# brdav/refign

Measured on AMD Instinct MI355X. Metric: image-pairs/s (align+seg fwd+bwd, 1080x1920), higher is better.
Workload: dtype bf16

## Files before the change

### include/refign_hip.h

```cpp
#ifndef REFIGN_HIP_H
#define REFIGN_HIP_H

#ifdef __cplusplus
extern "C" {
#endif

#define RFN_OK 0
#define RFN_EINVAL (-1)
#define RFN_ELAUNCH (-2)
#define RFN_ENOTSUP (-3)
#define RFN_ENONDET (-4)

#define RFN_ABI_VERSION 5

typedef void* rfn_stream_t;

int rfn_abi_version(void);
const char* rfn_last_error(void);

int rfn_set_deterministic(int on);
int rfn_get_deterministic(void);

int rfn_corr_fwd_f32(const float* in1, const float* in2, float* out, int B, int C, int iH, int iW,
                     int kH, int kW, int patchH, int patchW, int padH, int padW, int dilH, int dilW,
// ... 220 lines not shown
int rfn_dacs_blur(const float* x, float* tmp, float* y, int B, int C, int H, int W, int ksize_y, int ksize_x, const int* blur_on,
                  const double* sigma_y, const double* sigma_x, rfn_stream_t stream);

int rfn_crop_label_hist_u8(const void* label, int H, int W, const int* boxes, int K, int* hist, rfn_stream_t stream);
int rfn_crop_flip_norm_u8(const void* image, const void* label, int C, int H, int W, int top, int left, int h, int w, int flip,
                          const float* mean3, const float* std3, float* out_image, long* out_label, rfn_stream_t stream);

int rfn_resize_crop_flip_norm_u8(const void* image_hwc, int H, int W, int Hd, int Wd, const int* bounds_x, const int* coef_x, int kmax_x,
                                 const int* bounds_y, const int* coef_y, int kmax_y, int top, int left, int h, int w, int flip,
                                 const float* mean3, const float* std3, float* out_image, rfn_stream_t stream);
int rfn_resize_u8(const void* image_hwc, int H, int W, int Hd, int Wd, const int* bounds_x, const int* coef_x, int kmax_x,
                  const int* bounds_y, const int* coef_y, int kmax_y, void* out_chw, rfn_stream_t stream);
int rfn_resize_nearest_u8(const void* label, int H, int W, int Hd, int Wd, const int* ytab, const int* xtab, void* out,
                          rfn_stream_t stream);

int rfn_resize_filter_u8(const void* image_hwc, int H, int W, int Hd, int Wd, int filter, const int* bounds_x, const int* coef_x,
                         int kmax_x, const int* bounds_y, const int* coef_y, int kmax_y, void* out_chw, rfn_stream_t stream);
int rfn_resize_filter_crop_flip_norm_pad_u8(const void* image_hwc, int H, int W, int Hd, int Wd, int filter, const int* bounds_x,
                                            const int* coef_x, int kmax_x, const int* bounds_y, const int* coef_y, int kmax_y, int top,
                                            int left, int h, int w, int flip, const float* mean3, const float* std3, float* out_image,
                                            int Hf, int Wf, rfn_stream_t stream);

int rfn_sparse_epe_f32(const float* flow, const float* conf, const float* pts_src, const float* pts_trg, const int* offsets, int B,
                       int h, int w, double* rows, rfn_stream_t stream);

int rfn_gemm_nt_f8(const void* X8, const void* W8, const float* wscale, float x_scale, const void* bias, const void* res,
                   const float* rowscale, int rows_per_sample, int act, void* Y, int out_f8, float out_q, long M, long N,
                   long K, long ldx, long ldw, long ldy, rfn_stream_t stream);
int rfn_quant_rows_f8(const void* table, int nchunks, rfn_stream_t stream);
int rfn_quant_f8(const void* x_bf16, void* y8, long n, float q, rfn_stream_t stream);
int rfn_layernorm_fwd_f8(const void* x_bf16, const float* gamma, const float* beta, void* y8, long rows, int C, float eps,
                         float out_q, rfn_stream_t stream);
int rfn_dwconv3x3_gelu_nhwc_fwd_f8(const void* x8, const float* weight, const float* bias, void* y8, int B, int H, int W, int C,
                                   float x_scale, float out_q, rfn_stream_t stream);
int rfn_attn_pack_f8(const void* kv8, long batch_stride, long row_stride, int B, int heads, int Nkv, int nst, void* pack,
                     rfn_stream_t stream);
int rfn_attn_fwd_f8(const void* q8, long q_batch_stride, long q_row_stride, const void* pack, void* o8, long o_batch_stride,
                    long o_row_stride, int B, int heads, int Nq, int Nkv, int nst, float scale, float q_scale, float k_scale,
                    float v_scale, float out_q, rfn_stream_t stream);

unsigned long rfn_bn_stats_det_workspace_bytes(long T, int C);
int rfn_bn_stats_fwd_det(const void* x, double* sums, void* workspace, long T, int C, int dtype, rfn_stream_t stream);
int rfn_bn_stats_bwd_det(const void* x, const void* grad_y, const double* fwd_sums, const float* gamma, const float* beta,
                         float* bwd_sums, void* workspace, long T, int C, float eps, int relu, int dtype, rfn_stream_t stream);
unsigned long rfn_dwconv3x3_stats_det_workspace_bytes(int B, int H, int W, int C, int dilation);
int rfn_dwconv3x3_nhwc_fwd_stats_det(const void* x, const float* weight, const float* bias, void* y, double* sums, void* workspace,
                                     int B, int H, int W, int C, int dilation, int dtype, rfn_stream_t stream);
int rfn_dwconv3x3_nhwc_stats_det(const void* x, const float* weight, const float* bias, double* sums, void* workspace, int B, int H,
                                 int W, int C, int dilation, int dtype, rfn_stream_t stream);
int rfn_attn_bwd_dkv_det(const void* K, const void* V, long kv_batch_stride, long kv_row_stride, const void* q_rpack,
                         const void* q_tpack, const void* do_rpack, const void* do_tpack, const float* lse2,
                         const float* delta, float* accT, void* dKV, int B, int heads, int Nq, int Nkv, int nqblk, int nqpad,
                         int nkpad, int blocks_per_chunk, float scale, int dtype, rfn_stream_t stream);
unsigned long rfn_dacs_mix_jitter_det_workspace_bytes(int H, int W);
int rfn_dacs_mix_jitter_det(const float* src, const float* trg, const long* gt_src, const long* pseudo_label,
                            const float* pseudo_weight, float* mixed_img, long* mixed_lbl, float* mixed_weight, double* mean_ws,
                            int B, int H, int W, const long* class_bits, const int* jitter_on, const int* order,
                            const float* factor, const float* hue, const float* mean3, const float* std3,
                            rfn_stream_t stream);
unsigned long rfn_upsample_ce_det_workspace_bytes(int B, int C, int H, int W);
int rfn_upsample_ce_det(const void* logits, const long* target, const float* weight, float* grad_lo, double* loss_sum,
                        void* workspace, int B, int C, int h, int w, int H, int W, int ignore_index, int dtype, int round16,
                        rfn_stream_t stream);
int rfn_upsample_bilinear2d_bwd(const void* grad_out, void* grad_in, long planes, int h, int w, int H, int W, float scale_y,
                                float scale_x, int dtype, rfn_stream_t stream);

int rfn_steplog_gather(const void* const* ptrs, const int* dtypes, int n, double* row, rfn_stream_t stream);
int rfn_grad_sqnorm_groups(const float* flat, long n, const long* chunks, int nchunks, int ngroups, double* partials,
                           double* out, rfn_stream_t stream);

int rfn_flowsynth_flow_f32(const float* theta, int kind, const float* bumps, int n_bumps, const float* field, int h, int w,
                           float* flow, int* count, rfn_stream_t stream);
int rfn_flowsynth_warp_f32(const float* image, const float* flow, const int* count, int h, int w, int top, int left, int ch, int cw,
                           double min_fraction_valid, float* out_image, float* out_flow, void* out_mask, rfn_stream_t stream);
int rfn_gaussian_blur_f32(const float* src, const float* taps, int ntaps, int planes, int h, int w, double* tmp, float* dst,
                          rfn_stream_t stream);

int rfn_flowloss_block_pixels(void);
int rfn_flowloss_fwd_f32(const float* gt_flow, int B, int H, int W, const long* levels, const double* weights, int nlevels,
                         int loss_type, float delta, double* partials, int nblocks, float* loss_out, double* counts,
                         rfn_stream_t stream);
int rfn_flowloss_bwd_f32(const float* gt_flow, int B, int H, int W, const long* levels, const double* weights, int nlevels,
                         int loss_type, float delta, const double* counts, const float* grad_out, rfn_stream_t stream);
int rfn_multi_adam_f32(const void* table, int nchunks, const float* group_args, int ngroups, rfn_stream_t stream);
int rfn_multi_adam_amp_f32(const void* table, int nchunks, const double* group_args, int ngroups, const float* found_inf,
                           const float* step, rfn_stream_t stream);

int rfn_photometric_record_words(void);
int rfn_photometric_gray_sums_u8(const void* image, const void* records, int B, int h, int w, unsigned long* sums,
                                 rfn_stream_t stream);
int rfn_photometric_apply_u8(const void* image, const void* records, const unsigned long* sums, int B, int h, int w, float* out,
                             rfn_stream_t stream);

int rfn_rotate_nearest_u8(const void* src, int C, int H, int W, int a0, int a1, int a2, int a3, int a4, int a5, int fill,
                          void* out, void* outside, rfn_stream_t stream);
int rfn_photometric_gray_sums_geom_u8(const void* image, const void* records, const void* geom, int B, int H, int W, int h, int w,
                                      unsigned long* sums, rfn_stream_t stream);
int rfn_photometric_apply_geom_u8(const void* image, const void* records, const void* geom, const unsigned long* sums, int B, int H,
                                  int W, int h, int w, float* out, rfn_stream_t stream);

unsigned long rfn_warp_bwd_det_workspace_bytes(int B, int C, int H, int W, int want_grad_x, int want_grad_flow);
int rfn_warp_bwd_det_f32(const float* x, const float* flow, const float* grad_out, float* grad_x, float* grad_flow,
                         void* workspace, int B, int C, int H, int W, rfn_stream_t stream);
int rfn_corr_bwd_gather_f32(const float* in1, const float* in2, const float* grad_out, float* grad_in1,
                            float* grad_in2, int B, int C, int iH, int iW, int kH, int kW, int patchH, int patchW,
                            int padH, int padW, int dilH, int dilW, int dpH, int dpW, int dH, int dW,
// ... 7 lines not shown
```

### refign_amd/csrc/attn.hip

```cpp
#include <cstdlib>

#include "common.h"
#include "mfma.h"

namespace rfn {

constexpr int kPackBlock = 4096;
constexpr float kLog2e = 1.4426950408889634f;

__global__ __launch_bounds__(256) void attn_pack_kernel(const uint16_t* __restrict__ src0, const uint16_t* __restrict__ src1,
                                                        long sb, long sr, int heads, int nrows, int nblk,
                                                        unsigned char* __restrict__ rpack0, unsigned char* __restrict__ tpack0,
                                                        unsigned char* __restrict__ rpack1, unsigned char* __restrict__ tpack1) {
  __shared__ unsigned tile[32][33];
  const uint16_t* src = blockIdx.z ? src1 : src0;
  unsigned char* rpack = blockIdx.z ? rpack1 : rpack0;
  unsigned char* tpack = blockIdx.z ? tpack1 : tpack0;
  const int blk = blockIdx.x, bh = blockIdx.y;
  const int b = bh / heads, hd = bh % heads;
  const int t = threadIdx.x, row = t >> 3, dc = t & 7;
  const int grow = blk * 32 + row;
  u32x4 v = {0u, 0u, 0u, 0u};
  if (grow < nrows) v = *(const u32x4*)(src + (long)b * sb + (long)grow * sr + hd * 64 + dc * 8);
  unsigned char* rb = rpack + ((long)bh * nblk + blk) * kPackBlock;
// ... 144 lines not shown
      for (int kb = 0; kb < 2; ++kb)
#pragma unroll
        for (int r = 0; r < 16; ++r)
          if (key0 + kb * 32 + (r & 3) + 8 * (r >> 2) + 4 * g >= Nkv) p[kb][r] = -1e30f;
    }
    float mt = p[0][0];
#pragma unroll
    for (int kb = 0; kb < 2; ++kb)
#pragma unroll
      for (int r = 0; r < 16; ++r) mt = fmaxf(mt, p[kb][r]);
    mt = half_max(mt) * c;
    const float mnew = fmaxf(mrun, mt);
    if (__any(mnew > mrun)) {
      const float alpha = __builtin_amdgcn_exp2f(mrun - mnew);
      lrun *= alpha;
#pragma unroll
      for (int r = 0; r < 16; ++r) {
        oacc[0][r] *= alpha;
        oacc[1][r] *= alpha;
      }
      mrun = mnew;
    }
    float ps = 0.f;
#pragma unroll
    for (int kb = 0; kb < 2; ++kb)
#pragma unroll
      for (int r = 0; r < 16; ++r) {
        p[kb][r] = __builtin_amdgcn_exp2f(__builtin_fmaf(p[kb][r], c, -mrun));
        ps += p[kb][r];
      }
    lrun += ps;
    {
      vec8 pb[2][2];
      to_operands<DT>(p[0], pb[0]);
      to_operands<DT>(p[1], pb[1]);
#pragma unroll
      for (int idx = 0; idx < 8; ++idx) {
        const int kb = idx >> 2, m = (idx >> 1) & 1, db = idx & 1;
        oacc[db] = E::mma(vfr[idx & 3], pb[kb][m], oacc[db]);
        if (idx + 4 < 8) vfr[idx & 3] = vfrag(idx + 4);
        __builtin_amdgcn_sched_barrier(0);
      }
    }
    wait_dma_all();
    wg_barrier();
  }
  const float l = half_sum(lrun);
  const bool ok = q < Nq;
  store_rows64<DT>(oacc, 1.f / l, O + (long)b * osb + (long)(ok ? q : 0) * osr + hd * 64, ok, g);
  if (g == 0 && q < nqpad) lse2[(long)bh * nqpad + q] = ok ? mrun + log2f(l) : 0.f;
}


template <int DT>
__global__ __launch_bounds__(256) void attn_bwd_dq_kernel(const uint16_t* __restrict__ Q, long qsb, long qsr,
                                                          const uint16_t* __restrict__ dO, const uint16_t* __restrict__ O,
                                                          long osb, long osr, const unsigned char* __restrict__ Kr,
                                                          const unsigned char* __restrict__ Vr,
                                                          const unsigned char* __restrict__ Kt,
                                                          const float* __restrict__ lse2, float* __restrict__ delta,
                                                          uint16_t* __restrict__ dQ, long dsb, long dsr, int heads, int Nq,
                                                          int Nkv, int nblk, int nqpad, float scale, int pheads) {
  using E = Elem<DT>;
  using vec8 = typename E::vec8;
  constexpr int STAGE = 6 * kPackBlock;
  __shared__ __attribute__((aligned(16))) unsigned char smem[2 * STAGE];
  const int lane = threadIdx.x & 63, wave = threadIdx.x >> 6, g = lane >> 5, col = lane & 31;
  const int bh = blockIdx.y, b = bh / heads, hd = bh % heads;
  const int q = blockIdx.x * 128 + wave * 32 + col;
  const bool ok = q < Nq;
  const float c = scale * kLog2e;

  vec8 qf[4], gf[4];
  load_row_frags<DT>(Q + (long)b * qsb + hd * 64, qsr, q, Nq, g, qf);
  load_row_frags<DT>(dO + (long)b * osb + hd * 64, osr, q, Nq, g, gf);
  float dl = 0.f;
  {
    vec8 of[4];
    load_row_frags<DT>(O + (long)b * osb + hd * 64, osr, q, Nq, g, of);
#pragma unroll
    for (int kk = 0; kk < 4; ++kk)
#pragma unroll
      for (int e = 0; e < 8; ++e) dl += (float)gf[kk][e] * (float)of[kk][e];
    dl = half_sum(dl);
  }
  const float ls = (q < nqpad) ? lse2[(long)bh * nqpad + q] : 0.f;
  if (g == 0 && q < nqpad) delta[(long)bh * nqpad + q] = ok ? dl : 0.f;
#pragma unroll
  for (int kk = 0; kk < 4; ++kk) {
    pin_loaded(qf[kk]);
    pin_loaded(gf[kk]);
  }
  pin_loaded(ls);

  const long pbase = (long)(b * pheads + hd) * nblk * kPackBlock;
  const int nst = nblk / 2;
  auto issue = [&](int st, int buf) {
    unsigned char* dst = smem + buf * STAGE;
#pragma unroll
    for (int u = 0; u < 2; ++u) {
      const int piece = wave * 2 + u;
      const long off = pbase + (long)st * 2 * kPackBlock + piece * 1024 + lane * 16;
      lds_dma16(Kr + off, dst + piece * 1024);
      lds_dma16(Vr + off, dst + 2 * kPackBlock + piece * 1024);
      lds_dma16(Kt + off, dst + 4 * kPackBlock + piece * 1024);
    }
  };

  f32x16 dq[2];
#pragma unroll
  for (int r = 0; r < 16; ++r) dq[0][r] = dq[1][r] = 0.f;

  issue(0, 0);
  wait_dma_all();
  wg_barrier();
// ... 13 lines not shown
        const int kb = idx >> 3, kk = (idx >> 1) & 3;
        return *(const vec8*)(base + ((idx & 1) * 2 + kb) * kPackBlock + ((2 * kk + g) * 32 + col) * 16);
      };
#pragma unroll
      for (int idx = 0; idx < 4; ++idx) fr[idx] = frag(idx);
      __builtin_amdgcn_sched_barrier(0);
#pragma unroll
      for (int idx = 0; idx < 16; ++idx) {
        const int kb = idx >> 3, kk = (idx >> 1) & 3;
        if (idx & 1) dpacc[kb] = E::mma(fr[idx & 3], gf[kk], dpacc[kb]);
        else sacc[kb] = E::mma(fr[idx & 3], qf[kk], sacc[kb]);
        if (idx + 4 < 16) fr[idx & 3] = frag(idx + 4);
        __builtin_amdgcn_sched_barrier(0);
      }
    }
    vec8 ktf[4];
    auto ktfrag = [&](int idx) {
      const unsigned char* kq = base + (4 + (idx >> 2)) * kPackBlock + ((idx & 1) * 32 + col) * 8;
      const int m = (idx >> 1) & 1;
      return join8<DT>(*(const u32x2*)(kq + (4 * m + g) * 512), *(const u32x2*)(kq + (4 * m + 2 + g) * 512));
    };
#pragma unroll
    for (int idx = 0; idx < 4; ++idx) ktf[idx] = ktfrag(idx);
    __builtin_amdgcn_sched_barrier(0);
    float ds[2][16];
#pragma unroll
    for (int kb = 0; kb < 2; ++kb)
#pragma unroll
      for (int r = 0; r < 16; ++r)
        ds[kb][r] = __builtin_amdgcn_exp2f(__builtin_fmaf(sacc[kb][r], c, -ls)) * (dpacc[kb][r] - dl);
    if (key0 + 64 > Nkv) {
      asm volatile("; padded keys" ::: "memory");
#pragma unroll
      for (int kb = 0; kb < 2; ++kb)
#pragma unroll
        for (int r = 0; r < 16; ++r)
          if (key0 + kb * 32 + (r & 3) + 8 * (r >> 2) + 4 * g >= Nkv) ds[kb][r] = 0.f;
    }
    {
      vec8 sb[2][2];
      to_operands<DT>(ds[0], sb[0]);
      to_operands<DT>(ds[1], sb[1]);
#pragma unroll
      for (int idx = 0; idx < 8; ++idx) {
        dq[idx & 1] = E::mma(ktf[idx & 3], sb[idx >> 2][(idx >> 1) & 1], dq[idx & 1]);
        if (idx + 4 < 8) ktf[idx & 3] = ktfrag(idx + 4);
        __builtin_amdgcn_sched_barrier(0);
      }
    }
    wait_dma_all();
    wg_barrier();
  }
  store_rows64<DT>(dq, scale, dQ + (long)b * dsb + (long)(ok ? q : 0) * dsr + hd * 64, ok, g);
}

template <int DT, int NS>
__global__ __launch_bounds__(512) void attn_bwd_dkv_kernel(const uint16_t* __restrict__ K, const uint16_t* __restrict__ V,
                                                           long ksb, long ksr, const unsigned char* __restrict__ Qr,
                                                           const unsigned char* __restrict__ Qt,
                                                           const unsigned char* __restrict__ Gr,
                                                           const unsigned char* __restrict__ Gt,
                                                           const float* __restrict__ lse2, const float* __restrict__ delta,
                                                           float* __restrict__ accT, int heads, int Nq, int Nkv, int nqblk,
                                                           int nqpad, int nkpad, int blocks_per_chunk, float scale,
                                                           long chunk_stride = 0) {
  using E = Elem<DT>;
  using vec8 = typename E::vec8;
  constexpr int STATS = 4 * kPackBlock;
  constexpr int STAGE = STATS + 256;
  __shared__ __attribute__((aligned(16))) unsigned char smem[NS * STAGE];
  const int lane = threadIdx.x & 63, wave = threadIdx.x >> 6, g = lane >> 5, col = lane & 31;
  const int bh = blockIdx.z, b = bh / heads, hd = bh % heads;
  const int key = blockIdx.x * 256 + wave * 32 + col;
  const bool wave_live = blockIdx.x * 256 + wave * 32 < Nkv;
  const bool kok = key < Nkv;
  const float c = scale * kLog2e;

  vec8 kf[4], vf[4];
  load_row_frags<DT>(K + (long)b * ksb + hd * 64, ksr, key, Nkv, g, kf);
  load_row_frags<DT>(V + (long)b * ksb + hd * 64, ksr, key, Nkv, g, vf);
#pragma unroll
  for (int kk = 0; kk < 4; ++kk) {
    pin_loaded(kf[kk]);
    pin_loaded(vf[kk]);
  }

  const int qb0 = blockIdx.y * blocks_per_chunk;
  const int nst = min(qb0 + blocks_per_chunk, nqblk) - qb0;
  const long pbase = (long)bh * nqblk * kPackBlock;
  const float* stat_src = (g == 0 ? lse2 : delta) + (long)bh * nqpad + col;
  auto issue = [&](int qb, int buf) {
    unsigned char* dst = smem + buf * STAGE;
    const long off = pbase + (long)qb * kPackBlock + (wave & 3) * 1024 + lane * 16;
    if (wave < 4) {
      lds_dma16(Qr + off, dst + (wave & 3) * 1024);
      lds_dma16(Gr + off, dst + kPackBlock + (wave & 3) * 1024);
    } else {
      lds_dma16(Qt + off, dst + 2 * kPackBlock + (wave & 3) * 1024);
      lds_dma16(Gt + off, dst + 3 * kPackBlock + (wave & 3) * 1024);
    }
    if (wave == 0) lds_dma4(stat_src + qb * 32, dst + STATS);
  };

  f32x16 dk[2], dv[2];
#pragma unroll
  for (int r = 0; r < 16; ++r) dk[0][r] = dk[1][r] = dv[0][r] = dv[1][r] = 0.f;

#pragma unroll
  for (int s = 0; s < NS - 1; ++s)
    if (s < nst) issue(qb0 + s, s);
  for (int i = 0; i < nst; ++i) {
    if (NS == 2 || i + NS - 2 >= nst) wait_dma_all();
    else if (wave == 0) wait_dma_upto<(NS - 2) * 3>();
    else wait_dma_upto<(NS - 2) * 2>();
    wg_barrier();
    if (i + NS - 1 < nst) issue(qb0 + i + NS - 1, (i + NS - 1) % NS);
    if (wave_live) {
      const unsigned char* base = smem + (i % NS) * STAGE;
// ... 18 lines not shown
        for (int idx = 0; idx < 8; ++idx) {
          if (idx & 1) dp = E::mma(fr[idx & 3], vf[idx >> 1], dp);
          else s = E::mma(fr[idx & 3], kf[idx >> 1], s);
          if (idx + 4 < 8) fr[idx & 3] = frag(idx + 4);
          __builtin_amdgcn_sched_barrier(0);
        }
      }
      vec8 tf[4];
      auto tfrag = [&](int idx) {
        const int m = idx >> 2, db = (idx >> 1) & 1;
        const unsigned char* pq = base + (2 + ((idx & 1) ^ 1)) * kPackBlock + (db * 32 + col) * 8;
        return join8<DT>(*(const u32x2*)(pq + (4 * m + g) * 512), *(const u32x2*)(pq + (4 * m + 2 + g) * 512));
      };
#pragma unroll
      for (int idx = 0; idx < 4; ++idx) tf[idx] = tfrag(idx);
      __builtin_amdgcn_sched_barrier(0);
      float p[16], ds[16];
#pragma unroll
      for (int r = 0; r < 16; ++r) {
        float pr = __builtin_amdgcn_exp2f(__builtin_fmaf(s[r], c, -l4[r >> 2][r & 3]));
        if (!kok) pr = 0.f;
        p[r] = pr;
        ds[r] = pr * (dp[r] - d4[r >> 2][r & 3]);
      }
      vec8 pb[2], sb[2];
      to_operands<DT>(p, pb);
      to_operands<DT>(ds, sb);
#pragma unroll
      for (int idx = 0; idx < 8; ++idx) {
        const int m = idx >> 2, db = (idx >> 1) & 1;
        if (idx & 1) dk[db] = E::mma(tf[idx & 3], sb[m], dk[db]);
        else dv[db] = E::mma(tf[idx & 3], pb[m], dv[db]);
        if (idx + 4 < 8) tf[idx & 3] = tfrag(idx + 4);
        __builtin_amdgcn_sched_barrier(0);
      }
    }
  }
  if (kok) {
    float* ak = accT + (long)blockIdx.y * chunk_stride + (long)bh * 2 * 64 * nkpad + key;
    float* av = ak + (long)64 * nkpad;
#pragma unroll
    for (int db = 0; db < 2; ++db)
#pragma unroll
      for (int r = 0; r < 16; ++r) {
        const int d = db * 32 + (r & 3) + 8 * (r >> 2) + 4 * g;
        if (chunk_stride != 0) {
          ak[(long)d * nkpad] = dk[db][r] * scale;
          av[(long)d * nkpad] = dv[db][r];
        } else {
          atomicAdd(ak + (long)d * nkpad, dk[db][r] * scale);
          atomicAdd(av + (long)d * nkpad, dv[db][r]);
        }
      }
  }
}

template <int DT>
__global__ __launch_bounds__(256) void attn_dkv_finish_kernel(const float* __restrict__ accT, uint16_t* __restrict__ dkv,
                                                              int heads, int Nkv, int nkpad, long total, int chunks = 1,
                                                              long chunk_stride = 0) {
  using S = typename Elem<DT>::scalar;
  const long i = (long)blockIdx.x * 256 + threadIdx.x;
  if (i >= total) return;
  const int d = (int)(i & 63);
  long r = i >> 6;
  const int hd = (int)(r % heads);
  r /= heads;
  const int which = (int)(r & 1);
  r >>= 1;
  const int key = (int)(r % Nkv);
  const int b = (int)(r / Nkv);
  const float* p = accT + (((long)(b * heads + hd) * 2 + which) * 64 + d) * nkpad + key;
  float v = p[0];
  for (int c = 1; c < chunks; ++c) v += p[(long)c * chunk_stride];
  const S o = (S)v;
  dkv[i] = __builtin_bit_cast(uint16_t, o);
}

}

extern "C" {

using namespace rfn;

#define ATTN_DT_OK(dt) RFN_REQUIRE((dt) == 1 || (dt) == 2, "attention: dtype %d (1 = bf16, 2 = f16)", (dt))

int rfn_attn_pack(const void* src, long batch_stride, long row_stride, int B, int heads, int nrows, int nblk, void* rpack,
                  void* tpack, const void* src2, void* rpack2, void* tpack2, rfn_stream_t stream) {
  RFN_REQUIRE(src && (rpack || tpack), "attn_pack: null pointer");
  RFN_REQUIRE(src2 == nullptr || rpack2 || tpack2, "attn_pack: second tensor without outputs");
  RFN_REQUIRE(B > 0 && heads > 0 && nrows > 0 && nblk * 32 >= nrows, "attn_pack: B=%d heads=%d rows=%d nblk=%d", B, heads,
              nrows, nblk);
  RFN_REQUIRE(row_stride % 8 == 0 && batch_stride % 8 == 0, "attn_pack: strides must be multiples of 8 elements");
  dim3 grid(nblk, B * heads, src2 ? 2 : 1);
  hipLaunchKernelGGL(attn_pack_kernel, grid, dim3(256), 0, (hipStream_t)stream, (const uint16_t*)src,
                     (const uint16_t*)src2, batch_stride, row_stride, heads, nrows, nblk, (unsigned char*)rpack,
                     (unsigned char*)tpack, (unsigned char*)rpack2, (unsigned char*)tpack2);
  return check_launch("attn_pack");
}

int rfn_attn_fwd(const void* Q, long q_batch_stride, long q_row_stride, const void* k_rpack, const void* v_tpack, void* O,
                 long o_batch_stride, long o_row_stride, float* lse2, int B, int heads, int Nq, int Nkv, int nkblk,
                 int nqpad, float scale, int kv_pack_heads, int dtype, rfn_stream_t stream) {
  ATTN_DT_OK(dtype);
  RFN_REQUIRE(Q && k_rpack && v_tpack && O && lse2, "attn_fwd: null pointer");
  RFN_REQUIRE(B > 0 && heads > 0 && Nq > 0 && Nkv > 0 && nkblk % 2 == 0 && nkblk * 32 >= Nkv && nqpad >= Nq,
              "attn_fwd: B=%d heads=%d Nq=%d Nkv=%d nkblk=%d nqpad=%d", B, heads, Nq, Nkv, nkblk, nqpad);
  RFN_REQUIRE(q_row_stride % 8 == 0 && o_row_stride % 8 == 0 && q_batch_stride % 8 == 0 && o_batch_stride % 8 == 0,
              "attn_fwd: strides must be multiples of 8 elements");
  RFN_REQUIRE(kv_pack_heads >= heads, "attn_fwd: kv_pack_heads");
  dim3 grid(cdiv(Nq, 128), B * heads);
  if (dtype == 1)
    hipLaunchKernelGGL(attn_fwd_kernel<1>, grid, dim3(256), 0, (hipStream_t)stream, (const uint16_t*)Q, q_batch_stride,
                       q_row_stride, (const unsigned char*)k_rpack, (const unsigned char*)v_tpack, (uint16_t*)O,
                       o_batch_stride, o_row_stride, lse2, heads, Nq, Nkv, nkblk, nqpad, scale, kv_pack_heads);
  else
    hipLaunchKernelGGL(attn_fwd_kernel<2>, grid, dim3(256), 0, (hipStream_t)stream, (const uint16_t*)Q, q_batch_stride,
                       q_row_stride, (const unsigned char*)k_rpack, (const unsigned char*)v_tpack, (uint16_t*)O,
                       o_batch_stride, o_row_stride, lse2, heads, Nq, Nkv, nkblk, nqpad, scale, kv_pack_heads);
  return check_launch("attn_fwd");
}

int rfn_attn_bwd_dq(const void* Q, long q_batch_stride, long q_row_stride, const void* dO, const void* O,
                    long o_batch_stride, long o_row_stride, const void* k_rpack, const void* v_rpack, const void* k_tpack,
                    const float* lse2, float* delta, void* dQ, long dq_batch_stride, long dq_row_stride, int B, int heads,
                    int Nq, int Nkv, int nkblk, int nqpad, float scale, int kv_pack_heads, int dtype,
                    rfn_stream_t stream) {
  ATTN_DT_OK(dtype);
  RFN_REQUIRE(Q && dO && O && k_rpack && v_rpack && k_tpack && lse2 && delta && dQ, "attn_bwd_dq: null pointer");
  RFN_REQUIRE(B > 0 && heads > 0 && Nq > 0 && Nkv > 0 && nkblk % 2 == 0 && nkblk * 32 >= Nkv && nqpad >= Nq,
              "attn_bwd_dq: B=%d heads=%d Nq=%d Nkv=%d nkblk=%d nqpad=%d", B, heads, Nq, Nkv, nkblk, nqpad);
  dim3 grid(cdiv(Nq, 128), B * heads);
#define RFN_DQ_LAUNCH(D)                                                                                                \
  hipLaunchKernelGGL(attn_bwd_dq_kernel<D>, grid, dim3(256), 0, (hipStream_t)stream, (const uint16_t*)Q, q_batch_stride, \
                     q_row_stride, (const uint16_t*)dO, (const uint16_t*)O, o_batch_stride, o_row_stride,               \
                     (const unsigned char*)k_rpack, (const unsigned char*)v_rpack, (const unsigned char*)k_tpack, lse2,  \
                     delta, (uint16_t*)dQ, dq_batch_stride, dq_row_stride, heads, Nq, Nkv, nkblk, nqpad, scale,          \
                     kv_pack_heads)
  if (dtype == 1) RFN_DQ_LAUNCH(1); else RFN_DQ_LAUNCH(2);
#undef RFN_DQ_LAUNCH
  return check_launch("attn_bwd_dq");
}

static int attn_bwd_dkv_impl(bool det, const void* K, const void* V, long kv_batch_stride, long kv_row_stride, const void* q_rpack,
                             const void* q_tpack, const void* do_rpack, const void* do_tpack, const float* lse2,
                             const float* delta, float* accT, void* dKV, int B, int heads, int Nq, int Nkv, int nqblk, int nqpad,
                             int nkpad, int blocks_per_chunk, float scale, int dtype, rfn_stream_t stream) {
  ATTN_DT_OK(dtype);
  RFN_REQUIRE(K && V && q_rpack && q_tpack && do_rpack && do_tpack && lse2 && delta && accT && dKV,
              "attn_bwd_dkv: null pointer");
  RFN_REQUIRE(B > 0 && heads > 0 && Nq > 0 && Nkv > 0 && nqblk * 32 >= Nq && nqpad >= nqblk * 32 && nkpad >= Nkv &&
                  nkpad % 32 == 0 && blocks_per_chunk > 0,
              "attn_bwd_dkv: B=%d heads=%d Nq=%d Nkv=%d nqblk=%d nqpad=%d nkpad=%d chunk=%d", B, heads, Nq, Nkv, nqblk,
              nqpad, nkpad, blocks_per_chunk);
  hipStream_t s = (hipStream_t)stream;
  const long image = (long)B * heads * 2 * 64 * nkpad, chunk_stride = det ? image : 0;
  if (!det)
    if (int rc = zero_async(accT, (size_t)image * sizeof(float), s)) return rc;
  dim3 grid(cdiv(Nkv, 256), cdiv(nqblk, blocks_per_chunk), B * heads);
  const int chunks = det ? (int)grid.y : 1;
  static const int ring = 2;
#define RFN_DKV_LAUNCH_(D, R)                                                                                           \
  hipLaunchKernelGGL((attn_bwd_dkv_kernel<D, R>), grid, dim3(512), 0, s, (const uint16_t*)K, (const uint16_t*)V,            \
                     kv_batch_stride, kv_row_stride, (const unsigned char*)q_rpack, (const unsigned char*)q_tpack,      \
                     (const unsigned char*)do_rpack, (const unsigned char*)do_tpack, lse2, delta, accT, heads, Nq, Nkv,  \
                     nqblk, nqpad, nkpad, blocks_per_chunk, scale, chunk_stride)
#define RFN_DKV_LAUNCH(D)                                                                                               \
  switch (ring) {                                                                                                       \
    case 4: RFN_DKV_LAUNCH_(D, 4); break;                                                                               \
    default: RFN_DKV_LAUNCH_(D, 2); break;                                                                              \
  }
  if (dtype == 1) { RFN_DKV_LAUNCH(1) } else { RFN_DKV_LAUNCH(2) }
#undef RFN_DKV_LAUNCH
#undef RFN_DKV_LAUNCH_
  int rc = check_launch("attn_bwd_dkv");
  if (rc != RFN_OK) return rc;
  const long total = (long)B * Nkv * 2 * heads * 64;
  if (dtype == 1)
    hipLaunchKernelGGL(attn_dkv_finish_kernel<1>, dim3(cdiv(total, 256)), dim3(256), 0, s, accT, (uint16_t*)dKV, heads,
                       Nkv, nkpad, total, chunks, chunk_stride);
  else
    hipLaunchKernelGGL(attn_dkv_finish_kernel<2>, dim3(cdiv(total, 256)), dim3(256), 0, s, accT, (uint16_t*)dKV, heads,
                       Nkv, nkpad, total, chunks, chunk_stride);
  return check_launch("attn_dkv_finish");
}

int rfn_attn_bwd_dkv(const void* K, const void* V, long kv_batch_stride, long kv_row_stride, const void* q_rpack,
                     const void* q_tpack, const void* do_rpack, const void* do_tpack, const float* lse2,
                     const float* delta, float* accT, void* dKV, int B, int heads, int Nq, int Nkv, int nqblk, int nqpad,
                     int nkpad, int blocks_per_chunk, float scale, int dtype, rfn_stream_t stream) {
  RFN_REFUSE_NONDET(true, "rfn_attn_bwd_dkv", "attn_bwd_dkv_kernel, fp32 atomics (use rfn_attn_bwd_dkv_det)");
  return attn_bwd_dkv_impl(false, K, V, kv_batch_stride, kv_row_stride, q_rpack, q_tpack, do_rpack, do_tpack, lse2, delta, accT,
                           dKV, B, heads, Nq, Nkv, nqblk, nqpad, nkpad, blocks_per_chunk, scale, dtype, stream);
}

int rfn_attn_bwd_dkv_det(const void* K, const void* V, long kv_batch_stride, long kv_row_stride, const void* q_rpack,
                         const void* q_tpack, const void* do_rpack, const void* do_tpack, const float* lse2,
                         const float* delta, float* accT, void* dKV, int B, int heads, int Nq, int Nkv, int nqblk, int nqpad,
                         int nkpad, int blocks_per_chunk, float scale, int dtype, rfn_stream_t stream) {
  return attn_bwd_dkv_impl(true, K, V, kv_batch_stride, kv_row_stride, q_rpack, q_tpack, do_rpack, do_tpack, lse2, delta, accT,
                           dKV, B, heads, Nq, Nkv, nqblk, nqpad, nkpad, blocks_per_chunk, scale, dtype, stream);
}

}
```

### refign_amd/mfma.py

```python
import ctypes
import os

import torch

from . import _lib, determinism
from ._tensor import ptr
from ._tensor import DTYPE_CODE16 as _DT16

ENABLED = True

LIBRARY_CALLS = {}
_NOTE = True


def note_library(kind, *tensors):
    if not _NOTE or not tensors or not tensors[0].is_cuda:
        return
    key = (kind, str(tensors[0].dtype).replace("torch.", ""), tuple(tuple(t.shape) for t in tensors))
    n = LIBRARY_CALLS.get(key)
    if n is None and len(LIBRARY_CALLS) < 4096:
        if os.environ.get("RFN_LOG_LIBRARY", "0") == "1":
            print(f"[refign_amd] library fallback: {kind} {key[1]} {key[2]}", flush=True)
        LIBRARY_CALLS[key] = 1
    elif n is not None:
# ... 264 lines not shown
    @staticmethod
    def backward(ctx, g):
        flush_wgrads()
        return g


def wgrad_mark(x):
    return _WgradMark.apply(x) if (GROUP_WGRADS and torch.is_grad_enabled() and x.requires_grad) else x


_PACK_BLOCK = 4096


def _pack(src, batch_stride, row_stride, B, heads, nrows, nblk, want_r=True, want_t=True, src2=None):
    dev = src.device
    nbytes = B * heads * nblk * _PACK_BLOCK
    new = lambda want: torch.empty(nbytes, dtype=torch.uint8, device=dev) if want else None
    r, t = new(want_r), new(want_t)
    r2, t2 = (new(want_r), new(want_t)) if src2 is not None else (None, None)
    _lib.call("rfn_attn_pack", dev, ptr(src), batch_stride, row_stride, B, heads, nrows, nblk, ptr(r), ptr(t), ptr(src2),
              ptr(r2), ptr(t2))
    return (r, t), (r2, t2)


def _attn_ok(q, kv, heads):
    if not (ENABLED and q.is_cuda and q.dtype in _DT16 and kv.dtype == q.dtype and q.dim() == 3 and kv.dim() == 3):
        return False
    B, N, C = q.shape
    return (C == heads * 64 and kv.shape[0] == B and kv.shape[2] == 2 * C and q.is_contiguous() and kv.is_contiguous()
            and q.data_ptr() % 16 == 0 and kv.data_ptr() % 16 == 0)


def _dims(q, kv):
    B, N, C = q.shape
    Nkv = kv.shape[1]
    nkblk = -(-Nkv // 32)
    nkblk += nkblk & 1
    nqblk = -(-N // 32)
    return B, N, C, Nkv, nkblk, nqblk, nqblk * 32


def _fwd(q, kv, heads, scale, need_bwd):
    B, N, C, Nkv, nkblk, nqblk, nqpad = _dims(q, kv)
    dev = q.device
    (kvr, kvt), _ = _pack(kv, kv.stride(0), kv.stride(1), B, 2 * heads, Nkv, nkblk)
    voff = heads * nkblk * _PACK_BLOCK
    o = torch.empty_like(q)
    lse2 = torch.empty((B * heads, nqpad), dtype=torch.float32, device=dev)
    _lib.call("rfn_attn_fwd", dev, ptr(q), q.stride(0), q.stride(1), kvr.data_ptr(), kvt.data_ptr() + voff, ptr(o), o.stride(0),
              o.stride(1), ptr(lse2), B, heads, N, Nkv, nkblk, nqpad, float(scale), 2 * heads, _DT16[q.dtype])
    return o, lse2, (kvr, kvt)


def _chunk_blocks(nqblk, Nkv, BH):
    kblocks = -(-Nkv // 256)
    chunks = max(1, 128 // max(1, kblocks * BH))
    return max(4, -(-nqblk // chunks))


class _AttnFn(torch.autograd.Function):
    @staticmethod
    def forward(ctx, q, kv, heads, scale):
        need = q.requires_grad or kv.requires_grad
        o, lse2, packs = _fwd(q, kv, heads, scale, need)
        if need:
            ctx.save_for_backward(q, kv, o, lse2, *packs)
            ctx.heads, ctx.scale = heads, scale
        return o

    @staticmethod
    def backward(ctx, do):
        q, kv, o, lse2, kvr, kvt = ctx.saved_tensors
        heads, scale = ctx.heads, ctx.scale
        B, N, C, Nkv, nkblk, nqblk, nqpad = _dims(q, kv)
        dev = q.device
        if do.dtype != q.dtype:
            do = do.to(q.dtype)
        if not do.is_contiguous():
            do = do.contiguous()
        dt = _DT16[q.dtype]
        dq = torch.empty_like(q)
        delta = torch.empty_like(lse2)
        voff = heads * nkblk * _PACK_BLOCK
        _lib.call("rfn_attn_bwd_dq", dev, ptr(q), q.stride(0), q.stride(1), ptr(do), ptr(o), o.stride(0), o.stride(1),
                  kvr.data_ptr(), kvr.data_ptr() + voff, kvt.data_ptr(), ptr(lse2), ptr(delta), ptr(dq), dq.stride(0),
                  dq.stride(1), B, heads, N, Nkv, nkblk, nqpad, float(scale), 2 * heads, dt)
        (qr, qt), (gr, gt) = _pack(q, q.stride(0), q.stride(1), B, heads, N, nqblk, src2=do)
        nkpad = -(-Nkv // 32) * 32
        chunk = _chunk_blocks(nqblk, Nkv, B * heads)
        det = determinism.enabled()
        images = -(-nqblk // chunk) if det else 1
        accT = torch.empty(images * B * heads * 2 * 64 * nkpad, dtype=torch.float32, device=dev)
        dkv = torch.empty_like(kv)
        k_view, v_view = kv[:, :, :C], kv[:, :, C:]
        _lib.call("rfn_attn_bwd_dkv_det" if det else "rfn_attn_bwd_dkv", dev, ptr(k_view), ptr(v_view), kv.stride(0), kv.stride(1),
                  ptr(qr), ptr(qt), ptr(gr), ptr(gt), ptr(lse2), ptr(delta), ptr(accT), ptr(dkv), B, heads, N, Nkv, nqblk, nqpad,
                  nkpad, chunk, float(scale), dt)
        return dq, dkv, None, None


def attention(q, kv, heads, scale):
    if not _attn_ok(q, kv, heads):
        return None
    return _AttnFn.apply(q, kv, heads, scale)
```

Baseline: 16.73.

## Fuse Q/dO packing into dQ kernel and join dKV reduction via tickets

The dQ backward kernel now also writes the row- and transposed-packed layouts of Q and dO from fragments it already holds in registers, which removes the separate pack kernel launch and its re-read of Q and dO. The dKV kernel takes a last-arriver ticket scheme: the final chunk workgroup for each key tile sums the per-chunk fp32 images and writes bf16 dKV directly, replacing the separate reduction pass. The Python path now always uses the deterministic chunked images. In exchange it adds cross-workgroup atomics and fences, extra workspace, and changes the dQ grid to one workgroup per four query blocks.

Result: no change. 16.78 (median of 3 runs) (+0.3%).

```diff
diff --git a/include/refign_hip.h b/include/refign_hip.h
--- a/include/refign_hip.h
+++ b/include/refign_hip.h
@@ -296,6 +296,16 @@
                          const void* q_tpack, const void* do_rpack, const void* do_tpack, const float* lse2,
                          const float* delta, float* accT, void* dKV, int B, int heads, int Nq, int Nkv, int nqblk, int nqpad,
                          int nkpad, int blocks_per_chunk, float scale, int dtype, rfn_stream_t stream);
+int rfn_attn_bwd_dq_pack(const void* Q, long q_batch_stride, long q_row_stride, const void* dO, const void* O,
+                         long o_batch_stride, long o_row_stride, const void* k_rpack, const void* v_rpack, const void* k_tpack,
+                         const float* lse2, float* delta, void* dQ, long dq_batch_stride, long dq_row_stride, int B, int heads,
+                         int Nq, int Nkv, int nkblk, int nqpad, float scale, int kv_pack_heads, int dtype, void* q_rpack,
+                         void* q_tpack, void* do_rpack, void* do_tpack, int nqblk, unsigned* tickets, int n_tickets,
+                         rfn_stream_t stream);
+int rfn_attn_bwd_dkv_joined(const void* K, const void* V, long kv_batch_stride, long kv_row_stride, const void* q_rpack,
+                            const void* q_tpack, const void* do_rpack, const void* do_tpack, const float* lse2,
+                            const float* delta, float* accT, unsigned* tickets, void* dKV, int B, int heads, int Nq, int Nkv,
+                            int nqblk, int nqpad, int nkpad, int blocks_per_chunk, float scale, int dtype, rfn_stream_t stream);
 unsigned long rfn_dacs_mix_jitter_det_workspace_bytes(int H, int W);
 int rfn_dacs_mix_jitter_det(const float* src, const float* trg, const long* gt_src, const long* pseudo_label,
                             const float* pseudo_weight, float* mixed_img, long* mixed_lbl, float* mixed_weight, double* mean_ws,
diff --git a/refign_amd/csrc/attn.hip b/refign_amd/csrc/attn.hip
--- a/refign_amd/csrc/attn.hip
+++ b/refign_amd/csrc/attn.hip
@@ -220,7 +220,7 @@
 }
 
 
-template <int DT>
+template <int DT, bool PACK = false>
 __global__ __launch_bounds__(256) void attn_bwd_dq_kernel(const uint16_t* __restrict__ Q, long qsb, long qsr,
                                                           const uint16_t* __restrict__ dO, const uint16_t* __restrict__ O,
                                                           long osb, long osr, const unsigned char* __restrict__ Kr,
@@ -228,7 +228,12 @@
                                                           const unsigned char* __restrict__ Kt,
                                                           const float* __restrict__ lse2, float* __restrict__ delta,
                                                           uint16_t* __restrict__ dQ, long dsb, long dsr, int heads, int Nq,
-                                                          int Nkv, int nblk, int nqpad, float scale, int pheads) {
+                                                          int Nkv, int nblk, int nqpad, float scale, int pheads,
+                                                          unsigned char* __restrict__ Qr = nullptr,
+                                                          unsigned char* __restrict__ Qt = nullptr,
+                                                          unsigned char* __restrict__ Gr = nullptr,
+                                                          unsigned char* __restrict__ Gt = nullptr, int nqblk = 0,
+                                                          unsigned* __restrict__ tickets = nullptr, int n_tickets = 0) {
   using E = Elem<DT>;
   using vec8 = typename E::vec8;
   constexpr int STAGE = 6 * kPackBlock;
@@ -348,9 +353,44 @@
     wg_barrier();
   }
   store_rows64<DT>(dq, scale, dQ + (long)b * dsb + (long)(ok ? q : 0) * dsr + hd * 64, ok, g);
-}
-
-template <int DT, int NS>
+  if constexpr (PACK) {
+    if (blockIdx.x == 0 && blockIdx.y == 0)
+      for (int i = threadIdx.x; i < n_tickets; i += 256) tickets[i] = 0u;
+    const int blk = blockIdx.x * 4 + wave;
+    if (blk < nqblk) {
+      const long pb = ((long)bh * nqblk + blk) * kPackBlock;
+      static_assert(4 * 32 * 33 * 4 <= 2 * STAGE, "four tiles fit the ring");
+      unsigned* tile = (unsigned*)smem + wave * (32 * 33);
+      auto pack = [&](const vec8(&f)[4], unsigned char* rp, unsigned char* tp) {
+#pragma unroll
+        for (int kk = 0; kk < 4; ++kk) {
+          const u32x4 v = __builtin_bit_cast(u32x4, f[kk]);
+          *(u32x4*)(rp + pb + ((2 * kk + g) * 32 + col) * 16) = v;
+#pragma unroll
+          for (int j = 0; j < 4; ++j) tile[col * 33 + (2 * kk + g) * 4 + j] = v[j];
+        }
+        asm volatile("s_waitcnt lgkmcnt(0)" ::: "memory");
+#pragma unroll
+        for (int it = 0; it < 4; ++it) {
+          const int rq = 2 * it + g;
+          const unsigned r0 = tile[(4 * rq + 0) * 33 + col], r1 = tile[(4 * rq + 1) * 33 + col];
+          const unsigned r2 = tile[(4 * rq + 2) * 33 + col], r3 = tile[(4 * rq + 3) * 33 + col];
+          u32x4 o;
+          o[0] = (r0 & 0xffffu) | (r1 << 16);
+          o[1] = (r2 & 0xffffu) | (r3 << 16);
+          o[2] = (r0 >> 16) | (r1 & 0xffff0000u);
+          o[3] = (r2 >> 16) | (r3 & 0xffff0000u);
+          *(u32x4*)(tp + pb + (rq * 64 + 2 * col) * 8) = o;
+        }
+        asm volatile("s_waitcnt lgkmcnt(0)" ::: "memory");
+      };
+      pack(qf, Qr, Qt);
+      pack(gf, Gr, Gt);
+    }
+  }
+}
+
+template <int DT, int NS, bool JOIN = false>
 __global__ __launch_bounds__(512) void attn_bwd_dkv_kernel(const uint16_t* __restrict__ K, const uint16_t* __restrict__ V,
                                                            long ksb, long ksr, const unsigned char* __restrict__ Qr,
                                                            const unsigned char* __restrict__ Qt,
@@ -359,7 +399,8 @@
                                                            const float* __restrict__ lse2, const float* __restrict__ delta,
                                                            float* __restrict__ accT, int heads, int Nq, int Nkv, int nqblk,
                                                            int nqpad, int nkpad, int blocks_per_chunk, float scale,
-                                                           long chunk_stride = 0) {
+                                                           long chunk_stride = 0, unsigned* __restrict__ tickets = nullptr,
+                                                           uint16_t* __restrict__ dKV = nullptr) {
   using E = Elem<DT>;
   using vec8 = typename E::vec8;
   constexpr int STATS = 4 * kPackBlock;
@@ -484,6 +525,68 @@
           atomicAdd(av + (long)d * nkpad, dv[db][r]);
         }
       }
+  }
+  if constexpr (JOIN) {
+    using S = typename E::scalar;
+    constexpr int TILE = 2 * 32 * 33 * 4;
+    static_assert(2 * TILE + 16 <= NS * STAGE, "JOIN: the transpose tiles fit the ring");
+    asm volatile("s_waitcnt vmcnt(0)" ::: "memory");
+    __syncthreads();
+    int* flag = reinterpret_cast<int*>(smem + 2 * TILE);
+    if (threadIdx.x == 0) {
+      unsigned* tk = tickets + (long)bh * gridDim.x + blockIdx.x;
+      __builtin_amdgcn_fence(__ATOMIC_RELEASE, "agent");
+      asm volatile("s_waitcnt vmcnt(0)" ::: "memory");
+      const unsigned prev = __hip_atomic_fetch_add(tk, 1u, __ATOMIC_RELAXED, __HIP_MEMORY_SCOPE_AGENT);
+      const int last = prev == gridDim.y - 1;
+      if (last) {
+        __builtin_amdgcn_fence(__ATOMIC_ACQUIRE, "agent");
+        __hip_atomic_store(tk, 0u, __ATOMIC_RELAXED, __HIP_MEMORY_SCOPE_AGENT);
+      }
+      flag[0] = last;
+    }
+    __syncthreads();
+    const int last = flag[0];
+    __syncthreads();
+    if (!last) return;
+    const int chunks = (int)gridDim.y, t = threadIdx.x, d = t >> 3, k4 = t & 7;
+    const int ow = t >> 8, okey = (t >> 3) & 31, oc = t & 7;
+    const long vplane = (long)64 * nkpad;
+    const float* img = accT + ((long)bh * 2 * 64 + d) * nkpad + blockIdx.x * 256 + 4 * k4;
+    for (int p = 0; p < 8; ++p) {
+      const int key0 = blockIdx.x * 256 + p * 32;
+      if (key0 >= Nkv) break;
+      const float* src = img + p * 32;
+      f32x4 vk = *(const f32x4*)src, vv = *(const f32x4*)(src + vplane);
+      for (int c0 = 1; c0 < chunks; c0 += 8) {
+        f32x4 ak[8], av[8];
+#pragma unroll
+        for (int j = 0; j < 8; ++j) {
+          const float* q = src + (long)min(c0 + j, chunks - 1) * chunk_stride;
+          ak[j] = *(const f32x4*)q;
+          av[j] = *(const f32x4*)(q + vplane);
+        }
+#pragma unroll
+        for (int j = 0; j < 8; ++j)
+          if (c0 + j < chunks) {
+            vk += ak[j];
+            vv += av[j];
+          }
+      }
+      unsigned char* tl = smem + (p & 1) * TILE;
+      uint16_t* tw = reinterpret_cast<uint16_t*>(tl);
+#pragma unroll
+      for (int j = 0; j < 4; ++j) {
+        const S sk = (S)vk[j], sv = (S)vv[j];
+        tw[(4 * k4 + j) * 66 + d] = __builtin_bit_cast(uint16_t, sk);
+        tw[(32 + 4 * k4 + j) * 66 + d] = __builtin_bit_cast(uint16_t, sv);
+      }
+      __syncthreads();
+      const unsigned* rd = reinterpret_cast<const unsigned*>(tl) + (ow * 32 + okey) * 33 + oc * 4;
+      const u32x4 o = {rd[0], rd[1], rd[2], rd[3]};
+      const int key = key0 + okey;
+      if (key < Nkv) *(u32x4*)(dKV + ((((long)b * Nkv + key) * 2 + ow) * heads + hd) * 64 + oc * 8) = o;
+    }
   }
 }
 
@@ -553,29 +656,63 @@
   return check_launch("attn_fwd");
 }
 
+static int attn_bwd_dq_impl(bool pack, const void* Q, long q_batch_stride, long q_row_stride, const void* dO, const void* O,
+                           long o_batch_stride, long o_row_stride, const void* k_rpack, const void* v_rpack, const void* k_tpack,
+                           const float* lse2, float* delta, void* dQ, long dq_batch_stride, long dq_row_stride, int B, int heads,
+                           int Nq, int Nkv, int nkblk, int nqpad, float scale, int kv_pack_heads, int dtype, void* q_rpack,
+                           void* q_tpack, void* do_rpack, void* do_tpack, int nqblk, unsigned* tickets, int n_tickets,
+                           rfn_stream_t stream) {
+  ATTN_DT_OK(dtype);
+  RFN_REQUIRE(Q && dO && O && k_rpack && v_rpack && k_tpack && lse2 && delta && dQ, "attn_bwd_dq: null pointer");
+  RFN_REQUIRE(B > 0 && heads > 0 && Nq > 0 && Nkv > 0 && nkblk % 2 == 0 && nkblk * 32 >= Nkv && nqpad >= Nq,
+              "attn_bwd_dq: B=%d heads=%d Nq=%d Nkv=%d nkblk=%d nqpad=%d", B, heads, Nq, Nkv, nkblk, nqpad);
+  if (pack) {
+    RFN_REQUIRE(q_rpack && q_tpack && do_rpack && do_tpack, "attn_bwd_dq_pack: null pack pointer");
+    RFN_REQUIRE(nqblk * 32 >= Nq && n_tickets >= 0 && (tickets != nullptr || n_tickets == 0),
+                "attn_bwd_dq_pack: Nq=%d nqblk=%d n_tickets=%d", Nq, nqblk, n_tickets);
+    RFN_REQUIRE(q_row_stride % 8 == 0 && q_batch_stride % 8 == 0 && o_row_stride % 8 == 0 && o_batch_stride % 8 == 0,
+                "attn_bwd_dq_pack: strides must be multiples of 8 elements");
+  }
+  dim3 grid(pack ? cdiv(nqblk, 4) : cdiv(Nq, 128), B * heads);
+#define RFN_DQ_LAUNCH(D, P)                                                                                              \
+  hipLaunchKernelGGL((attn_bwd_dq_kernel<D, P>), grid, dim3(256), 0, (hipStream_t)stream, (const uint16_t*)Q,             \
+                     q_batch_stride, q_row_stride, (const uint16_t*)dO, (const uint16_t*)O, o_batch_stride, o_row_stride, \
+                     (const unsigned char*)k_rpack, (const unsigned char*)v_rpack, (const unsigned char*)k_tpack, lse2,   \
+                     delta, (uint16_t*)dQ, dq_batch_stride, dq_row_stride, heads, Nq, Nkv, nkblk, nqpad, scale,           \
+                     kv_pack_heads, (unsigned char*)q_rpack, (unsigned char*)q_tpack, (unsigned char*)do_rpack,           \
+                     (unsigned char*)do_tpack, nqblk, tickets, n_tickets)
+  if (pack) {
+    if (dtype == 1) RFN_DQ_LAUNCH(1, true); else RFN_DQ_LAUNCH(2, true);
+  } else {
+    if (dtype == 1) RFN_DQ_LAUNCH(1, false); else RFN_DQ_LAUNCH(2, false);
+  }
+#undef RFN_DQ_LAUNCH
+  return check_launch(pack ? "attn_bwd_dq_pack" : "attn_bwd_dq");
+}
+
 int rfn_attn_bwd_dq(const void* Q, long q_batch_stride, long q_row_stride, const void* dO, const void* O,
                     long o_batch_stride, long o_row_stride, const void* k_rpack, const void* v_rpack, const void* k_tpack,
                     const float* lse2, float* delta, void* dQ, long dq_batch_stride, long dq_row_stride, int B, int heads,
                     int Nq, int Nkv, int nkblk, int nqpad, float scale, int kv_pack_heads, int dtype,
                     rfn_stream_t stream) {
-  ATTN_DT_OK(dtype);
-  RFN_REQUIRE(Q && dO && O && k_rpack && v_rpack && k_tpack && lse2 && delta && dQ, "attn_bwd_dq: null pointer");
-  RFN_REQUIRE(B > 0 && heads > 0 && Nq > 0 && Nkv > 0 && nkblk % 2 == 0 && nkblk * 32 >= Nkv && nqpad >= Nq,
-              "attn_bwd_dq: B=%d heads=%d Nq=%d Nkv=%d nkblk=%d nqpad=%d", B, heads, Nq, Nkv, nkblk, nqpad);
-  dim3 grid(cdiv(Nq, 128), B * heads);
-#define RFN_DQ_LAUNCH(D)                                                                                                \
-  hipLaunchKernelGGL(attn_bwd_dq_kernel<D>, grid, dim3(256), 0, (hipStream_t)stream, (const uint16_t*)Q, q_batch_stride, \
-                     q_row_stride, (const uint16_t*)dO, (const uint16_t*)O, o_batch_stride, o_row_stride,               \
-                     (const unsigned char*)k_rpack, (const unsigned char*)v_rpack, (const unsigned char*)k_tpack, lse2,  \
-                     delta, (uint16_t*)dQ, dq_batch_stride, dq_row_stride, heads, Nq, Nkv, nkblk, nqpad, scale,          \
-                     kv_pack_heads)
-  if (dtype == 1) RFN_DQ_LAUNCH(1); else RFN_DQ_LAUNCH(2);
-#undef RFN_DQ_LAUNCH
-  return check_launch("attn_bwd_dq");
-}
-
-static int attn_bwd_dkv_impl(bool det, const void* K, const void* V, long kv_batch_stride, long kv_row_stride, const void* q_rpack,
-                             const void* q_tpack, const void* do_rpack, const void* do_tpack, const float* lse2,
+  return attn_bwd_dq_impl(false, Q, q_batch_stride, q_row_stride, dO, O, o_batch_stride, o_row_stride, k_rpack, v_rpack, k_tpack,
+                          lse2, delta, dQ, dq_batch_stride, dq_row_stride, B, heads, Nq, Nkv, nkblk, nqpad, scale, kv_pack_heads,
+                          dtype, nullptr, nullptr, nullptr, nullptr, 0, nullptr, 0, stream);
+}
+
+int rfn_attn_bwd_dq_pack(const void* Q, long q_batch_stride, long q_row_stride, const void* dO, const void* O,
+                         long o_batch_stride, long o_row_stride, const void* k_rpack, const void* v_rpack, const void* k_tpack,
+                         const float* lse2, float* delta, void* dQ, long dq_batch_stride, long dq_row_stride, int B, int heads,
+                         int Nq, int Nkv, int nkblk, int nqpad, float scale, int kv_pack_heads, int dtype, void* q_rpack,
+                         void* q_tpack, void* do_rpack, void* do_tpack, int nqblk, unsigned* tickets, int n_tickets,
+                         rfn_stream_t stream) {
+  return attn_bwd_dq_impl(true, Q, q_batch_stride, q_row_stride, dO, O, o_batch_stride, o_row_stride, k_rpack, v_rpack, k_tpack,
+                          lse2, delta, dQ, dq_batch_stride, dq_row_stride, B, heads, Nq, Nkv, nkblk, nqpad, scale, kv_pack_heads,
+                          dtype, q_rpack, q_tpack, do_rpack, do_tpack, nqblk, tickets, n_tickets, stream);
+}
+
+static int attn_bwd_dkv_impl(bool det, unsigned* tickets, const void* K, const void* V, long kv_batch_stride, long kv_row_stride,
+                             const void* q_rpack, const void* q_tpack, const void* do_rpack, const void* do_tpack, const float* lse2,
                              const float* delta, float* accT, void* dKV, int B, int heads, int Nq, int Nkv, int nqblk, int nqpad,
                              int nkpad, int blocks_per_chunk, float scale, int dtype, rfn_stream_t stream) {
   ATTN_DT_OK(dtype);
@@ -591,20 +728,17 @@
     if (int rc = zero_async(accT, (size_t)image * sizeof(float), s)) return rc;
   dim3 grid(cdiv(Nkv, 256), cdiv(nqblk, blocks_per_chunk), B * heads);
   const int chunks = det ? (int)grid.y : 1;
-  static const int ring = 2;
-#define RFN_DKV_LAUNCH_(D, R)                                                                                           \
-  hipLaunchKernelGGL((attn_bwd_dkv_kernel<D, R>), grid, dim3(512), 0, s, (const uint16_t*)K, (const uint16_t*)V,            \
+#define RFN_DKV_LAUNCH(D, J)                                                                                             \
+  hipLaunchKernelGGL((attn_bwd_dkv_kernel<D, 2, J>), grid, dim3(512), 0, s, (const uint16_t*)K, (const uint16_t*)V,       \
                      kv_batch_stride, kv_row_stride, (const unsigned char*)q_rpack, (const unsigned char*)q_tpack,      \
                      (const unsigned char*)do_rpack, (const unsigned char*)do_tpack, lse2, delta, accT, heads, Nq, Nkv,  \
-                     nqblk, nqpad, nkpad, blocks_per_chunk, scale, chunk_stride)
-#define RFN_DKV_LAUNCH(D)                                                                                               \
-  switch (ring) {                                                                                                       \
-    case 4: RFN_DKV_LAUNCH_(D, 4); break;                                                                               \
-    default: RFN_DKV_LAUNCH_(D, 2); break;                                                                              \
-  }
-  if (dtype == 1) { RFN_DKV_LAUNCH(1) } else { RFN_DKV_LAUNCH(2) }
+                     nqblk, nqpad, nkpad, blocks_per_chunk, scale, chunk_stride, tickets, (uint16_t*)dKV)
+  if (tickets != nullptr) {
+    if (dtype == 1) RFN_DKV_LAUNCH(1, true); else RFN_DKV_LAUNCH(2, true);
+    return check_launch("attn_bwd_dkv_joined");
+  }
+  if (dtype == 1) RFN_DKV_LAUNCH(1, false); else RFN_DKV_LAUNCH(2, false);
 #undef RFN_DKV_LAUNCH
-#undef RFN_DKV_LAUNCH_
   int rc = check_launch("attn_bwd_dkv");
   if (rc != RFN_OK) return rc;
   const long total = (long)B * Nkv * 2 * heads * 64;
@@ -622,7 +756,7 @@
                      const float* delta, float* accT, void* dKV, int B, int heads, int Nq, int Nkv, int nqblk, int nqpad,
                      int nkpad, int blocks_per_chunk, float scale, int dtype, rfn_stream_t stream) {
   RFN_REFUSE_NONDET(true, "rfn_attn_bwd_dkv", "attn_bwd_dkv_kernel, fp32 atomics (use rfn_attn_bwd_dkv_det)");
-  return attn_bwd_dkv_impl(false, K, V, kv_batch_stride, kv_row_stride, q_rpack, q_tpack, do_rpack, do_tpack, lse2, delta, accT,
+  return attn_bwd_dkv_impl(false, nullptr, K, V, kv_batch_stride, kv_row_stride, q_rpack, q_tpack, do_rpack, do_tpack, lse2, delta, accT,
                            dKV, B, heads, Nq, Nkv, nqblk, nqpad, nkpad, blocks_per_chunk, scale, dtype, stream);
 }
 
@@ -630,8 +764,17 @@
                          const void* q_tpack, const void* do_rpack, const void* do_tpack, const float* lse2,
                          const float* delta, float* accT, void* dKV, int B, int heads, int Nq, int Nkv, int nqblk, int nqpad,
                          int nkpad, int blocks_per_chunk, float scale, int dtype, rfn_stream_t stream) {
-  return attn_bwd_dkv_impl(true, K, V, kv_batch_stride, kv_row_stride, q_rpack, q_tpack, do_rpack, do_tpack, lse2, delta, accT,
+  return attn_bwd_dkv_impl(true, nullptr, K, V, kv_batch_stride, kv_row_stride, q_rpack, q_tpack, do_rpack, do_tpack, lse2, delta, accT,
                            dKV, B, heads, Nq, Nkv, nqblk, nqpad, nkpad, blocks_per_chunk, scale, dtype, stream);
 }
 
-}
+int rfn_attn_bwd_dkv_joined(const void* K, const void* V, long kv_batch_stride, long kv_row_stride, const void* q_rpack,
+                            const void* q_tpack, const void* do_rpack, const void* do_tpack, const float* lse2,
+                            const float* delta, float* accT, unsigned* tickets, void* dKV, int B, int heads, int Nq, int Nkv,
+                            int nqblk, int nqpad, int nkpad, int blocks_per_chunk, float scale, int dtype, rfn_stream_t stream) {
+  RFN_REQUIRE(tickets != nullptr, "attn_bwd_dkv_joined: null tickets");
+  return attn_bwd_dkv_impl(true, tickets, K, V, kv_batch_stride, kv_row_stride, q_rpack, q_tpack, do_rpack, do_tpack, lse2, delta,
+                           accT, dKV, B, heads, Nq, Nkv, nqblk, nqpad, nkpad, blocks_per_chunk, scale, dtype, stream);
+}
+
+}
diff --git a/refign_amd/mfma.py b/refign_amd/mfma.py
--- a/refign_amd/mfma.py
+++ b/refign_amd/mfma.py
@@ -340,9 +340,12 @@
     return o, lse2, (kvr, kvt)
 
 
+_DKV_WORKGROUPS = 128
+
+
 def _chunk_blocks(nqblk, Nkv, BH):
     kblocks = -(-Nkv // 256)
-    chunks = max(1, 128 // max(1, kblocks * BH))
+    chunks = max(1, _DKV_WORKGROUPS // max(1, kblocks * BH))
     return max(4, -(-nqblk // chunks))
 
 
@@ -370,20 +373,23 @@
         dq = torch.empty_like(q)
         delta = torch.empty_like(lse2)
         voff = heads * nkblk * _PACK_BLOCK
-        _lib.call("rfn_attn_bwd_dq", dev, ptr(q), q.stride(0), q.stride(1), ptr(do), ptr(o), o.stride(0), o.stride(1),
-                  kvr.data_ptr(), kvr.data_ptr() + voff, kvt.data_ptr(), ptr(lse2), ptr(delta), ptr(dq), dq.stride(0),
-                  dq.stride(1), B, heads, N, Nkv, nkblk, nqpad, float(scale), 2 * heads, dt)
-        (qr, qt), (gr, gt) = _pack(q, q.stride(0), q.stride(1), B, heads, N, nqblk, src2=do)
+        nbytes = B * heads * nqblk * _PACK_BLOCK
+        packs = torch.empty(4 * nbytes, dtype=torch.uint8, device=dev)
+        qr, qt, gr, gt = (packs.data_ptr() + i * nbytes for i in range(4))
         nkpad = -(-Nkv // 32) * 32
         chunk = _chunk_blocks(nqblk, Nkv, B * heads)
-        det = determinism.enabled()
-        images = -(-nqblk // chunk) if det else 1
+        images = -(-nqblk // chunk)
         accT = torch.empty(images * B * heads * 2 * 64 * nkpad, dtype=torch.float32, device=dev)
+        tickets = torch.empty(B * heads * -(-Nkv // 256), dtype=torch.int32, device=dev)
+        _lib.call("rfn_attn_bwd_dq_pack", dev, ptr(q), q.stride(0), q.stride(1), ptr(do), ptr(o), o.stride(0), o.stride(1),
+                  kvr.data_ptr(), kvr.data_ptr() + voff, kvt.data_ptr(), ptr(lse2), ptr(delta), ptr(dq), dq.stride(0),
+                  dq.stride(1), B, heads, N, Nkv, nkblk, nqpad, float(scale), 2 * heads, dt, qr, qt, gr, gt,
+                  nqblk, ptr(tickets), tickets.numel())
         dkv = torch.empty_like(kv)
         k_view, v_view = kv[:, :, :C], kv[:, :, C:]
-        _lib.call("rfn_attn_bwd_dkv_det" if det else "rfn_attn_bwd_dkv", dev, ptr(k_view), ptr(v_view), kv.stride(0), kv.stride(1),
-                  ptr(qr), ptr(qt), ptr(gr), ptr(gt), ptr(lse2), ptr(delta), ptr(accT), ptr(dkv), B, heads, N, Nkv, nqblk, nqpad,
-                  nkpad, chunk, float(scale), dt)
+        _lib.call("rfn_attn_bwd_dkv_joined", dev, ptr(k_view), ptr(v_view), kv.stride(0), kv.stride(1), qr, qt, gr,
+                  gt, ptr(lse2), ptr(delta), ptr(accT), ptr(tickets), ptr(dkv), B, heads, N, Nkv, nqblk, nqpad, nkpad, chunk,
+                  float(scale), dt)
         return dq, dkv, None, None
 
 
```
